# dfm/george

Hardware: NVIDIA H100
Metric: gp.compute+log_likelihood N-points/sec (higher is better)
Workload: dtype f64

## Files before the change

george_b200/csrc/hodlr.cu:

```cuda
#include <algorithm>
#include <cmath>
#include <cstdlib>
#include <cstring>
#include <vector>

#include "common.cuh"
#include "hodlr_kernels.cuh"
#include "hodlr_lu.cuh"
#include "hodlr_aca2.cuh"
#include "hodlr_leaf.cuh"
#include "linalg.cuh"
#include "kernel_eval.cuh"

namespace bgp {
int upload_program(const DevProgram& P, DevBuf<DevProgram>& buf, cudaStream_t s);
int kmat_grad_contract_launch(const DevProgram* dprog, int nd, int np, const unsigned* which_dev, const double* x,
                              int64_t n, const double* M, int64_t ldm, const double* alpha, double ca, double cm,
                              double* g_dev, double* diag_dev, DevBuf<double>& scratch, cudaStream_t s);
int fill_identity_launch(double* A, int64_t n, cudaStream_t s);
int64_t grad_slab_partial_size(int64_t n, int64_t c, int np);
int64_t grad_slab_tile_size(int64_t n, int np);
int kmat_grad_slab_launch(const DevProgram* dprog, int nd, int np, const unsigned* which_dev, const double* x, int64_t n,
                          const double* W, int64_t j0, int64_t nc, int64_t jlo, int64_t jhi, const double* alpha,
                          double* partial, double* tile_part, double* diag_dev, cudaStream_t s);
int kmat_grad_slab_finish(int np, int64_t jlo, int64_t jhi, const double* tile_part, double* g_dev, cudaStream_t s);
int kmat_symmetric_launch_auto(const DevProgram& P, const DevProgram* dprog, const double* x, int64_t n,
                               const double* diag_add, double* out, int64_t ld, cudaStream_t s);
int kmat_general_launch_auto(const DevProgram& P, const DevProgram* dprog, const double* x1, int64_t n1, const double* x2,
                             int64_t n2, double* out, int64_t ld, cudaStream_t s);
int kmat_diagonal_launch(const DevProgram* dprog, const double* x1, const double* x2, int64_t n, double* out,
                         cudaStream_t s, int members = 1, int64_t ostride = 0);
int64_t predict_chunk_cols(int64_t n, int64_t multiple);
int64_t predict_var_partial_size(int64_t n, int64_t c);
int predict_var_launch(const double* B, int64_t ldb, const double* W, int64_t ldw, int64_t n, int64_t c,
                       const double* kdiag, double* var, DevBuf<double>& scratch, cudaStream_t s);
int kmat_x1_grad_matvec_launch(const DevProgram& P, const DevProgram* dprog, const double* x1, int64_t n1,
                               const double* x2, int64_t n2, const double* V, int64_t ldv, double scale, int add_prior,
                               double* out, DevBuf<double>& scratch, cudaStream_t s);
int64_t x1_grad_partial_size(int64_t n1, int64_t n2, int nd);
void predict_gemm_plan(int64_t m, int64_t nn, int64_t K, int64_t* nsplit_out, int64_t* klen_out);
int predict_gemm_sub(const double* A, int64_t lda, const double* B, int64_t ldb, int64_t m, int64_t nn, int64_t K,
                     bool lower, double* C, int64_t ldc, DevBuf<double>& slices, DevBuf<GemmDesc>& descs, cudaStream_t s);
bool comm_ready();
int comm_rank();
int comm_world();
int comm_allreduce_sum_f64(double* buf, size_t count, cudaStream_t s);
int comm_allgather_f64(const double* send, double* recv, size_t count, cudaStream_t s);
}
using namespace bgp;

struct HNode {
  int start, size, half, is_leaf, parent, dir, depth;
  int slot;
  int rank = 0, draws = 0, fallback = 0;
  int owned = 1;
  int top = 0;
};

struct PanelSet {
  DevBuf<double> V, U;
  int64_t ld = 0, row_off = 0;
  int vcols = 0, ucols = 0;
  double* vbase() const { return V.p - row_off; }
  double* ubase() const { return U.p - row_off; }
};

struct LevelInfo {
  std::vector<int> nodes;
  int set = 1;
  int cap = 0, max_cap = 0, vcol = 0, r = 0, ucol = 0;
  int max_half = 0, grow = 0;
  int desc_off = 0;
};

struct AcaGraphKey {
  A2Args a;
  int nn, ncc, nrc, shape, grid;
};

struct bgp_hodlr {
  cudaStream_t sA = nullptr, sB = nullptr;
  cudaEvent_t ev[8] = {nullptr};
  int64_t n = 0;
  int ndim = 0;
  bgp_hodlr_opts_t opts;
  bool computed = false;
  double log_det = 0.0;
  DevProgram prog;

  std::vector<HNode> nodes;
  std::vector<int> leaves;
  std::vector<LevelInfo> levels;
  std::vector<int> piv_off;
  std::vector<int> h_piv_rows, h_piv_cols;
  int max_leaf = 0, rtot = 0, vcols = 0, cut_depth = 0;
  int64_t row0 = 0, nloc = 0;
  std::vector<int64_t> shard_row0, shard_rows;
  bool top_pending = false;

  DevBuf<DevProgram> d_prog;
  DevBuf<double> d_x, d_yerr, d_diag, d_L, d_leaf_logdet, d_node_logdet, d_S, d_W, d_scalar, d_rhs;
  PanelSet top, loc;
  const PanelSet& pset(const LevelInfo& L) const { return L.set == 0 ? top : loc; }
  DevBuf<double> d_inv, d_gscratch;
  DevBuf<double> d_xsend, d_xrecv;
  DevBuf<unsigned> d_which;
  LuWorkspace lu_ws;
  DevBuf<GemmDesc> d_gram_desc, d_upd_desc;
  std::vector<NodeDesc> h_nodes;
  std::vector<int> cap_hint;
  int64_t cap_hint_n = -1;
  int cap_hint_min_size = -1;
  DevBuf<LeafDesc> d_leaves;
  DevBuf<AcaDesc> d_aca;
  DevBuf<AcaOut> d_aca_out;
  DevBuf<NodeDesc> d_nodes;
  DevBuf<PanelTile> d_ptiles;
  int small_limit = SS_MAX_N;
  bool leaf_cols_wide = false;
  DevBuf<int> d_idx, d_piv_rows, d_piv_cols, d_ticket, d_chain_done, d_ncols_by_depth;
  DevBuf<uint32_t> d_chain_state;
  DevBuf<A2Node> d_a2nodes;
  DevBuf<A2State> d_a2states;
  DevBuf<MT19937> d_a2rngs;
  DevBuf<A2EPart> d_epart;
  DevBuf<int> d_cand, d_cand_k, d_cand_words, d_cand_L, d_cand_next, d_cand_live, d_cchunk_node, d_rchunk_node, d_nactive;
  DevBuf<double> d_node_box;
  DevBuf<double2> d_cand_xu, d_gbox, d_cbox;
  DevBuf<unsigned long long> d_cmax, d_stats;
  DevBuf<int4> d_work;
  DevBuf<int> d_work_count, d_iter;
  AcaGraphKey aca_key;
  cudaGraph_t aca_graph = nullptr;
  cudaGraphExec_t aca_exec = nullptr;
  cudaStream_t sC = nullptr;
  bool profile = false;
  std::vector<cudaEvent_t> prof_events;
  double prof[12] = {0, 0, 0, 0, 0, 0, 0, 0, 0, 0, 0, 0};
  uint64_t draw_paths[4] = {0, 0, 0, 0};
  uint64_t eval_units[2] = {0, 0};
  DevBuf<double> d_vpart, d_upart, d_vmax;
  int aca_iters = 0;
  size_t w_cap = 0;

  double t_ms[5] = {0, 0, 0, 0, 0};
  double grad_t[4] = {0, 0, 0, 0};
  double work[6] = {0, 0, 0, 0, 0, 0};
};

static int ensure_streams(bgp_hodlr* h) {
  if (!h->sA) {
    BGP_CUDA(cudaStreamCreateWithFlags(&h->sA, cudaStreamNonBlocking));
    BGP_CUDA(cudaStreamCreateWithFlags(&h->sB, cudaStreamNonBlocking));
    for (int i = 0; i < 8; ++i) BGP_CUDA(cudaEventCreate(&h->ev[i]));
  }
  return BGP_OK;
}

static void build_tree(bgp_hodlr* h, int start, int size, int dir, int parent, int depth) {
  HNode nd;
  nd.start = start; nd.size = size; nd.half = size / 2; nd.dir = dir; nd.parent = parent; nd.depth = depth;
  nd.is_leaf = !(nd.half >= h->opts.min_size);
  nd.slot = 0;
  const int id = (int)h->nodes.size();
  h->nodes.push_back(nd);
  if (!nd.is_leaf) {
    build_tree(h, start, nd.half, 0, id, depth + 1);
    build_tree(h, start + nd.half, size - nd.half, 1, id, depth + 1);
  }
}

static int hodlr_solve_dev(bgp_hodlr* h, double* b, int64_t nrhs, int64_t ldb, cudaStream_t s, int part,
                           int64_t eye_row0 = -1);
static int hodlr_exchange_finish(bgp_hodlr* h);

static bool host_exchange(const bgp_hodlr* h) {
  return h->opts.shard_count > 1 &&
         !(comm_ready() && comm_world() == h->opts.shard_count && comm_rank() == h->opts.shard_rank);
}

static int reject_host_exchange(const bgp_hodlr* h, const char* what) {
  if (!host_exchange(h)) return BGP_OK;
  set_error("%s is not available on a host-exchange shard (shard %d of %d without a matching communicator): use "
            "bgp_hodlr_solve_local_dev / bgp_hodlr_solve_top_dev", what, h->opts.shard_rank, h->opts.shard_count);
  return BGP_ERR_INVALID;
}
static int hodlr_finish_top_impl(bgp_hodlr* h, bool allreduce);

constexpr size_t LS_SMEM_MAX = 200 * 1024;
constexpr int LS_MAX_LEAF = (int)(LS_SMEM_MAX / sizeof(double));

static bool leaf_solve_fits(int max_leaf, int cols) { return sizeof(double) * (size_t)max_leaf * cols <= LS_SMEM_MAX; }

static void set_sweep_func_attrs() {
  static std::atomic<uint64_t> done{0};
  int dev = 0;
  cudaGetDevice(&dev);
  const uint64_t bit = dev < 64 ? (1ull << dev) : 0;
  if (bit && (done.load(std::memory_order_relaxed) & bit)) return;
  cudaFuncSetAttribute(leaf_solve_kernel<1>, cudaFuncAttributeMaxDynamicSharedMemorySize, (int)LS_SMEM_MAX);
  cudaFuncSetAttribute(leaf_solve_kernel<2>, cudaFuncAttributeMaxDynamicSharedMemorySize, (int)LS_SMEM_MAX);
  cudaFuncSetAttribute(leaf_solve_kernel<4>, cudaFuncAttributeMaxDynamicSharedMemorySize, (int)LS_SMEM_MAX);
  cudaFuncSetAttribute(leaf_solve_kernel<LS_COLS>, cudaFuncAttributeMaxDynamicSharedMemorySize, (int)LS_SMEM_MAX);
  cudaFuncSetAttribute(leaf_solve_kernel<LS_COLS_WIDE>, cudaFuncAttributeMaxDynamicSharedMemorySize, (int)LS_SMEM_MAX);
  cudaFuncSetAttribute(small_solve_kernel, cudaFuncAttributeMaxDynamicSharedMemorySize, 160 * 1024);
  done.fetch_or(bit, std::memory_order_relaxed);
}

template <int COLS>
static int leaf_solve_launch(bgp_hodlr* h, double* X, int64_t ldx, const int* ncols_by_depth, int ncols_fixed,
                             int max_cols, cudaStream_t s, int l0, int l1) {
  const int ngroups = (max_cols + COLS - 1) / COLS;
  const dim3 grid((unsigned)((size_t)(l1 - l0) * (size_t)ngroups));
  const size_t smem = sizeof(double) * (size_t)h->max_leaf * COLS;
  leaf_solve_kernel<COLS><<<grid, LS_THREADS, smem, s>>>(h->d_leaves.p + l0, h->d_L.p, X, ldx, ncols_by_depth,
                                                         ncols_fixed, h->max_leaf, ngroups);
  BGP_LAUNCH_CHECK();
  return BGP_OK;
}

static int launch_leaf_solve(bgp_hodlr* h, double* X, int64_t ldx, const int* ncols_by_depth, int ncols_fixed,
                             int max_cols, cudaStream_t s, int l0 = 0, int l1 = -1) {
  if (l1 < 0) l1 = (int)h->leaves.size();
  const int nl = l1 - l0;
  if (nl <= 0 || max_cols == 0) return BGP_OK;
  const int m = h->max_leaf;
  if (h->leaf_cols_wide && max_cols > LS_COLS && leaf_solve_fits(m, LS_COLS_WIDE))
    return leaf_solve_launch<LS_COLS_WIDE>(h, X, ldx, ncols_by_depth, ncols_fixed, max_cols, s, l0, l1);
  int cols = max_cols <= 1 ? 1 : max_cols <= 2 ? 2 : max_cols <= 4 ? 4 : LS_COLS;
  while (cols > 1 && !leaf_solve_fits(m, cols)) cols /= 2;
  if (!leaf_solve_fits(m, cols)) {
    set_error("leaf size %d too large for the leaf solve kernel (at most %d rows)", m, LS_MAX_LEAF);
    return BGP_ERR_INVALID;
  }
  switch (cols) {
    case LS_COLS: return leaf_solve_launch<LS_COLS>(h, X, ldx, ncols_by_depth, ncols_fixed, max_cols, s, l0, l1);
    case 4: return leaf_solve_launch<4>(h, X, ldx, ncols_by_depth, ncols_fixed, max_cols, s, l0, l1);
    case 2: return leaf_solve_launch<2>(h, X, ldx, ncols_by_depth, ncols_fixed, max_cols, s, l0, l1);
    default: return leaf_solve_launch<1>(h, X, ldx, ncols_by_depth, ncols_fixed, max_cols, s, l0, l1);
  }
}

static int launch_level_big(bgp_hodlr* h, const LevelInfo& L, double* X, int64_t ldx, int ncolsW, int own_off, int factor,
                            int col_lo, int col_hi, cudaStream_t s, int b0, int b1);

static int launch_level(bgp_hodlr* h, const LevelInfo& L, double* X, int64_t ldx, int ncolsW, int own_off, int factor,
                        int col_lo, int col_hi, cudaStream_t s, int b0 = 0, int b1 = -1) {
  if (b1 < 0) b1 = (int)L.nodes.size();
  const int nn = b1 - b0;
  if (nn <= 0 || L.r == 0) {
    return BGP_OK;
  }
  const int r = L.r;
  const int64_t stride = (int64_t)2 * r * ncolsW;
  const size_t need = (size_t)nn * stride;
  if (need > h->w_cap) { set_error("internal: W workspace too small (%zu > %zu)", need, h->w_cap); return BGP_ERR_CUDA; }
  BGP_CUDA(cudaMemsetAsync(h->d_W.p, 0, sizeof(double) * need, s));
  if (2 * r > h->small_limit) return launch_level_big(h, L, X, ldx, ncolsW, own_off, factor, col_lo, col_hi, s, b0, b1);
  const NodeDesc* nd = h->d_nodes.p + L.desc_off + b0;
  const int max_nh = L.max_half + 1;
  if (r <= GTS_MAX_R) {
    dim3 grid((max_nh + GTS_ROWS - 1) / GTS_ROWS, nn * 2, (ncolsW + GTS_TC - 1) / GTS_TC);
    const double* vb = h->pset(L).vbase();
    const int64_t ldv = h->pset(L).ld;
    if (r <= 2) gram_tn_small_kernel<2><<<grid, GTS_THREADS, 0, s>>>(nd, vb, ldv, X, ldx, ncolsW, h->d_W.p, stride);
    else if (r <= 4) gram_tn_small_kernel<4><<<grid, GTS_THREADS, 0, s>>>(nd, vb, ldv, X, ldx, ncolsW, h->d_W.p, stride);
    else gram_tn_small_kernel<GTS_MAX_R><<<grid, GTS_THREADS, 0, s>>>(nd, vb, ldv, X, ldx, ncolsW, h->d_W.p, stride);
    BGP_LAUNCH_CHECK();
  } else {
    dim3 grid((max_nh + GT_CHUNK - 1) / GT_CHUNK, nn * 2, (ncolsW + GT_TC - 1) / GT_TC);
    gram_tn_kernel<<<grid, GT_THREADS, 0, s>>>(nd, h->pset(L).vbase(), h->pset(L).ld, X, ldx, ncolsW, h->d_W.p, stride);
    BGP_LAUNCH_CHECK();
  }
  {
    const size_t sbytes = sizeof(double) * (size_t)(2 * r) * (2 * r);
    small_solve_kernel<<<nn, SS_THREADS, sbytes, s>>>(nd, h->d_W.p, stride, ncolsW, own_off, factor, h->d_S.p,
                                                      h->d_node_logdet.p, L.desc_off + b0);
    BGP_LAUNCH_CHECK();
  }
  if (col_hi > col_lo) {
    dim3 grid((max_nh + UP_ROWS - 1) / UP_ROWS, nn * 2, (col_hi - col_lo + UP_TC - 1) / UP_TC);
    update_nn_kernel<<<grid, UP_THREADS, 0, s>>>(nd, h->pset(L).ubase(), h->pset(L).ld, X, ldx, col_lo, col_hi, h->d_W.p, stride, 0);
    BGP_LAUNCH_CHECK();
  }
  return BGP_OK;
}

static int launch_level_big(bgp_hodlr* h, const LevelInfo& L, double* X, int64_t ldx, int ncolsW, int own_off, int factor,
                            int col_lo, int col_hi, cudaStream_t s, int b0, int b1) {
  const int nn = b1 - b0;
  const int r = L.r, n2 = 2 * r;
  const int64_t stride = (int64_t)n2 * ncolsW;
  const int64_t ldv = h->pset(L).ld, ldu = h->pset(L).ld;
  double* W = h->d_W.p;
  constexpr int KCHUNK = 4096;
  std::vector<LuNode> lun(nn);
  std::vector<GemmDesc> gram, upd;
  int max_nh = 0;
  for (int k = 0; k < nn; ++k) {
    const int b = b0 + k;
    const HNode& nd = h->nodes[L.nodes[b]];
    const int64_t s_off = h->h_nodes[L.desc_off + b].s_off;
    lun[k].S = h->d_S.p + s_off;
    lun[k].piv = reinterpret_cast<int*>(lun[k].S + (int64_t)n2 * n2);
    lun[k].logdet = h->d_node_logdet.p + L.desc_off + b;
    double* Wn = W + (int64_t)k * stride;
    for (int hh = 0; hh < 2; ++hh) {
      const int rs = nd.start + (hh ? nd.half : 0), nh = hh ? (nd.size - nd.half) : nd.half;
      max_nh = std::max(max_nh, nh);
      for (int k0 = 0; k0 < nh; k0 += KCHUNK) {
        GemmDesc g;
        g.A = h->pset(L).vbase() + (int64_t)L.vcol * ldv + rs + k0; g.lda = ldv;
        g.B = X + rs + k0; g.ldb = ldx;
        g.C = Wn + (hh ? 0 : r); g.ldc = n2;
        g.M = r; g.N = ncolsW; g.K = std::min(KCHUNK, nh - k0); g.mode = GD_ATOMIC_ADD;
        gram.push_back(g);
      }
      if (col_hi > col_lo) {
        GemmDesc g;
        g.A = h->pset(L).ubase() + (int64_t)L.ucol * ldu + rs; g.lda = ldu;
        g.B = Wn + (hh ? r : 0) + (int64_t)col_lo * n2; g.ldb = n2;
        g.C = X + rs + (int64_t)col_lo * ldx; g.ldc = ldx;
        g.M = nh; g.N = col_hi - col_lo; g.K = r; g.mode = GD_SUB;
        upd.push_back(g);
      }
    }
  }
  BGP_TRY(lu_upload(h->d_gram_desc, gram, s));
  BGP_TRY((gemm_dmma_launch<true, true>(h->d_gram_desc.p, (int)gram.size(), r, ncolsW, nullptr, s)));
  if (factor) {
    BGP_TRY(lu_upload(h->lu_ws.d_nodes, lun, s));
    dim3 grid((unsigned)std::min<int64_t>(((int64_t)n2 * n2 + 255) / 256, 4096), nn);
    lu_assemble_kernel<<<grid, 256, 0, s>>>(h->lu_ws.d_nodes.p, W, stride, r, own_off);
    BGP_LAUNCH_CHECK();
    BGP_TRY(lu_factor_batch(h->lu_ws, lun, n2, s));
    if (col_hi > col_lo)
      BGP_TRY(lu_solve_batch(h->lu_ws, lun, n2, W + (int64_t)col_lo * n2, stride, n2, col_hi - col_lo, false, s));
  } else {
    BGP_TRY(lu_solve_batch(h->lu_ws, lun, n2, W, stride, n2, ncolsW, true, s));
  }
  if (!upd.empty()) {
    BGP_TRY(lu_upload(h->d_upd_desc, upd, s));
    BGP_TRY((gemm_dmma_launch<false, true>(h->d_upd_desc.p, (int)upd.size(), max_nh, col_hi - col_lo, nullptr, s)));
  }
  return BGP_OK;
}

static int run_aca2(bgp_hodlr* h, const std::vector<AcaDesc>& descs, std::vector<AcaOut>& houts, cudaStream_t s) {
  const int nn = (int)descs.size();
  if (nn == 0) return BGP_OK;
  std::vector<A2Node> hn(nn);
  std::vector<int> cchunk_node, rchunk_node;
  int64_t cand_total = 0, top_cand_total = 0;
  (void)top_cand_total;
  const bool dist_top = false;
  int capmax = 1;
  for (int i = 0; i < nn; ++i) {
    const AcaDesc& d = descs[i];
    A2Node& a = hn[i];
    a.row0 = d.row0; a.n_rows = d.n_rows; a.col0 = d.col0; a.n_cols = d.n_cols;
    a.vcol = d.vcol; a.cap = d.cap; a.pre_id = d.pre_id; a.node = d.node;
    {
      const PanelSet& ps = h->pset(h->levels[h->nodes[d.pre_id].depth]);
      a.ld = ps.ld;
      a.vbase = ps.vbase() + (int64_t)d.vcol * ps.ld;
    }
    a.idx_off = d.idx_off; a.piv_off = d.piv_off;
    a.cchunk0 = (int)cchunk_node.size(); a.n_cchunks = (d.n_cols + A2_CHUNK - 1) / A2_CHUNK;
    a.rchunk0 = (int)rchunk_node.size(); a.n_rchunks = (d.n_rows + A2_CHUNK - 1) / A2_CHUNK;
    for (int c = 0; c < a.n_cchunks; ++c) cchunk_node.push_back(i);
    for (int c = 0; c < a.n_rchunks; ++c) rchunk_node.push_back(i);
    a.bmax = std::min(A2_BMAX, d.n_rows);
    a.cand_off = cand_total; cand_total += a.bmax;
    a.is_top = (dist_top && h->nodes[d.pre_id].top) ? 1 : 0;
    if (a.is_top) top_cand_total = cand_total;
    capmax = std::max(capmax, d.cap);
  }
  const int ncc = (int)cchunk_node.size(), nrc = (int)rchunk_node.size();
  BGP_TRY(h->d_a2nodes.reserve(nn, s));
  BGP_TRY(h->d_a2states.reserve(nn, s));
  BGP_TRY(h->d_a2rngs.reserve((size_t)2 * nn, s));
  BGP_TRY(h->d_cand.reserve((size_t)cand_total, s));
  BGP_TRY(h->d_cand_k.reserve((size_t)cand_total, s));
  BGP_TRY(h->d_cand_words.reserve((size_t)cand_total, s));
  BGP_TRY(h->d_cand_L.reserve((size_t)cand_total, s));
  BGP_TRY(h->d_cand_next.reserve((size_t)cand_total, s));
  BGP_TRY(h->d_cand_live.reserve((size_t)cand_total, s));
  BGP_TRY(h->d_node_box.reserve((size_t)2 * nn, s));
  BGP_TRY(h->d_cmax.reserve((size_t)cand_total, s));
  BGP_TRY(h->d_epart.reserve((size_t)std::max(ncc, 1) * A2_NSUB, s));
  BGP_TRY(h->d_cchunk_node.reserve(ncc, s));
  BGP_TRY(h->d_rchunk_node.reserve(nrc, s));
  BGP_TRY(h->d_vpart.reserve((size_t)ncc * A2_NSUB * (capmax + 1), s));
  BGP_TRY(h->d_upart.reserve((size_t)nrc * A2_NSUB * (capmax + 1), s));
  const bool cull = shape_has_bound(h->prog.shape) && !getenv("BGP_NO_CULL");
  if (cull) {
    BGP_TRY(h->d_vmax.reserve((size_t)ncc * A2_NGROUP, s));
    BGP_CUDA(cudaMemsetAsync(h->d_vmax.p, 0, sizeof(double) * ncc * A2_NGROUP, s));
    BGP_TRY(h->d_cand_xu.reserve((size_t)cand_total, s));
    BGP_TRY(h->d_gbox.reserve((size_t)ncc * A2_NGROUP, s));
    BGP_TRY(h->d_cbox.reserve((size_t)ncc, s));
  }
  BGP_TRY(h->d_nactive.reserve(2, s));
  int n_top = 0;
  for (int i = 0; i < nn; ++i) n_top += hn[i].is_top;
  BGP_TRY(h->d_stats.reserve(A2_NSTATS, s));
  int64_t work_cap = 0;
  for (int i = 0; i < nn; ++i) {
    const int big = (hn[i].bmax + A2_CG * A2_ITEM_CB - 1) / (A2_CG * A2_ITEM_CB);
    const int small = (std::min(hn[i].bmax, 256) + A2_CG - 1) / A2_CG;
    work_cap += (int64_t)hn[i].n_cchunks * std::max(big, small);
  }
  BGP_TRY(h->d_work.reserve((size_t)(2 * work_cap), s));
  BGP_TRY(h->d_work_count.reserve(4, s));
  BGP_TRY(h->d_iter.reserve(1, s));
  BGP_CUDA(cudaMemsetAsync(h->d_iter.p, 0, sizeof(int), s));
  BGP_CUDA(cudaMemsetAsync(h->d_work_count.p, 0, sizeof(int) * 4, s));
  BGP_CUDA(cudaMemsetAsync(h->d_stats.p, 0, sizeof(unsigned long long) * A2_NSTATS, s));
  BGP_CUDA(cudaMemcpyAsync(h->d_a2nodes.p, hn.data(), sizeof(A2Node) * nn, cudaMemcpyHostToDevice, s));
  BGP_CUDA(cudaMemcpyAsync(h->d_cchunk_node.p, cchunk_node.data(), sizeof(int) * ncc, cudaMemcpyHostToDevice, s));
  BGP_CUDA(cudaMemcpyAsync(h->d_rchunk_node.p, rchunk_node.data(), sizeof(int) * nrc, cudaMemcpyHostToDevice, s));
  BGP_CUDA(cudaMemcpyAsync(h->d_nactive.p, &nn, sizeof(int), cudaMemcpyHostToDevice, s));
  A2Args a;
  memset(&a, 0, sizeof(a));
  a.prog = h->d_prog.p; a.x = h->d_x.p; a.nodes = h->d_a2nodes.p; a.states = h->d_a2states.p; a.rngs = h->d_a2rngs.p; a.n_nodes = nn;
  a.tol = h->opts.tol; a.seed = (uint32_t)h->opts.seed; a.exhaust_mode = h->opts.exhaust_mode;
  a.idx_ws = h->d_idx.p; a.piv_rows = h->d_piv_rows.p; a.piv_cols = h->d_piv_cols.p;
  a.cand = h->d_cand.p; a.cand_k = h->d_cand_k.p; a.cand_words = h->d_cand_words.p; a.cmax = h->d_cmax.p; a.epart = h->d_epart.p;
  a.cchunk_node = h->d_cchunk_node.p; a.rchunk_node = h->d_rchunk_node.p; a.vpart = h->d_vpart.p; a.upart = h->d_upart.p;
  a.vmax = cull ? h->d_vmax.p : nullptr;
  a.cand_xu = cull ? h->d_cand_xu.p : nullptr;
  a.gbox = cull ? h->d_gbox.p : nullptr;
  a.cbox = cull ? h->d_cbox.p : nullptr;
  a.cand_L = h->d_cand_L.p; a.cand_next = h->d_cand_next.p; a.cand_live = h->d_cand_live.p; a.node_box = h->d_node_box.p;
  a.capmax = capmax; a.n_active = h->d_nactive.p; a.stats = h->d_stats.p;
  a.work = h->d_work.p; a.work_count = h->d_work_count.p; a.work_cursor = h->d_work_count.p + 2; a.work_cap = (int)work_cap; a.iter_ptr = h->d_iter.p;
  a.shard_rank = dist_top ? h->opts.shard_rank : 0; a.shard_count = dist_top ? h->opts.shard_count : 1;
  if (dist_top) BGP_CUDA(cudaMemcpyAsync(h->d_nactive.p + 1, &n_top, sizeof(int), cudaMemcpyHostToDevice, s));
  cudaFuncSetAttribute(a2_init_kernel, cudaFuncAttributeMaxDynamicSharedMemorySize, (int)sizeof(A2NodeSmem));
    cudaFuncSetAttribute(a2_decide_kernel, cudaFuncAttributeMaxDynamicSharedMemorySize, (int)sizeof(A2NodeSmem));
    cudaFuncSetAttribute(a2_finish_kernel, cudaFuncAttributeMaxDynamicSharedMemorySize, (int)sizeof(A2NodeSmem));
  a2_init_kernel<<<nn, A2_NODE_THREADS, sizeof(A2NodeSmem), s>>>(a);
  BGP_LAUNCH_CHECK();
  int active = nn, iters = 0;
  int eval_minb = A2_EVAL_MINB_DEFAULT;
  if (const char* e = getenv("BGP_EVAL_MINB")) eval_minb = atoi(e) == 3 ? 3 : 2;
  const int eval_grid = num_sms() * 6;
  auto launch_iteration = [&](cudaStream_t st, cudaGraphConditionalHandle hnd, int use_hnd, int it_prof) -> int {
    auto mark = [&](int slot) -> int {
      if (it_prof < 0) return BGP_OK;
      const size_t need = (size_t)7 * (it_prof + 1);
      while (h->prof_events.size() < need) {
        cudaEvent_t e;
        BGP_CUDA(cudaEventCreate(&e));
        h->prof_events.push_back(e);
      }
      BGP_CUDA(cudaEventRecord(h->prof_events[(size_t)7 * it_prof + slot], st));
      return BGP_OK;
    };
    BGP_TRY(mark(0));
    a2_eval_launch(h->prog.shape, dim3(eval_grid), st, a, eval_minb);
    BGP_LAUNCH_CHECK();
    BGP_TRY(mark(1));
    a2_decide_kernel<<<nn, A2_NODE_THREADS, sizeof(A2NodeSmem), st>>>(a);
    BGP_LAUNCH_CHECK();
    BGP_TRY(mark(2));
    a2_vrow_launch(h->prog.shape, dim3(ncc, A2_NSUB), st, a);
    BGP_LAUNCH_CHECK();
    BGP_TRY(mark(3));
    a2_pivot_kernel<<<nn, 32, 0, st>>>(a);
    BGP_LAUNCH_CHECK();
    BGP_TRY(mark(4));
    a2_vnorm_ucol_launch(h->prog.shape, dim3(ncc + nrc, A2_NSUB), st, a, ncc);
    BGP_LAUNCH_CHECK();
    BGP_TRY(mark(5));
    a2_finish_kernel<<<nn, A2_NODE_THREADS, sizeof(A2NodeSmem), st>>>(a);
    BGP_LAUNCH_CHECK();
    BGP_TRY(mark(6));
    a2_tick_kernel<<<1, 1, 0, st>>>(a.iter_ptr, a.n_active, hnd, use_hnd);
    BGP_LAUNCH_CHECK();
    return BGP_OK;
  };
  const bool use_graph = !h->profile && !getenv("BGP_NO_GRAPH");
  if (use_graph) {
    AcaGraphKey key;
    memset(&key, 0, sizeof(key));
    key.a = a; key.nn = nn; key.ncc = ncc; key.nrc = nrc; key.shape = h->prog.shape; key.grid = eval_grid * 4 + eval_minb;
    if (!h->aca_exec || memcmp(&key, &h->aca_key, sizeof(key)) != 0) {
      if (h->aca_exec) { cudaGraphExecDestroy(h->aca_exec); h->aca_exec = nullptr; }
      if (h->aca_graph) { cudaGraphDestroy(h->aca_graph); h->aca_graph = nullptr; }
      BGP_CUDA(cudaGraphCreate(&h->aca_graph, 0));
      cudaGraphConditionalHandle hnd;
      BGP_CUDA(cudaGraphConditionalHandleCreate(&hnd, h->aca_graph, 1, cudaGraphCondAssignDefault));
      cudaGraphNodeParams cp = {};
      cp.type = cudaGraphNodeTypeConditional;
      cp.conditional.handle = hnd;
      cp.conditional.type = cudaGraphCondTypeWhile;
      cp.conditional.size = 1;
      cudaGraphNode_t wnode;
      BGP_CUDA(cudaGraphAddNode(&wnode, h->aca_graph, nullptr, 0, &cp));
      cudaGraph_t body = cp.conditional.phGraph_out[0];
      if (!h->sC) BGP_CUDA(cudaStreamCreateWithFlags(&h->sC, cudaStreamNonBlocking));
      BGP_CUDA(cudaStreamBeginCaptureToGraph(h->sC, body, nullptr, nullptr, 0, cudaStreamCaptureModeRelaxed));
      const int rc = launch_iteration(h->sC, hnd, 1, -1);
      cudaGraph_t captured = nullptr;
      const cudaError_t ce = cudaStreamEndCapture(h->sC, &captured);
      if (rc != BGP_OK) return rc;
      if (ce != cudaSuccess) { set_error("ACA graph capture failed: %s", cudaGetErrorString(ce)); return BGP_ERR_CUDA; }
      BGP_CUDA(cudaGraphInstantiate(&h->aca_exec, h->aca_graph, 0));
      h->aca_key = key;
    }
    BGP_CUDA(cudaGraphLaunch(h->aca_exec, s));
    int it_host = 0, act2[2] = {0, 0};
    BGP_CUDA(cudaMemcpyAsync(&it_host, h->d_iter.p, sizeof(int), cudaMemcpyDeviceToHost, s));
    BGP_CUDA(cudaMemcpyAsync(act2, h->d_nactive.p, sizeof(int) * 2, cudaMemcpyDeviceToHost, s));
    BGP_CUDA(cudaStreamSynchronize(s));
    iters = it_host;
// ... 1329 lines not shown
```

george_b200/csrc/hodlr_kernels.cuh:

```cuda
#pragma once

#include <cooperative_groups.h>

#include "common.cuh"
#include "kernel_eval.cuh"

namespace bgp {

namespace cg = cooperative_groups;

struct MT19937 {
  uint32_t mt[624];
  int idx;
};
__device__ inline void mt_seed(MT19937& g, uint32_t s) {
  g.mt[0] = s;
  for (int i = 1; i < 624; ++i) g.mt[i] = 1812433253u * (g.mt[i - 1] ^ (g.mt[i - 1] >> 30)) + (uint32_t)i;
  g.idx = 624;
}
__device__ inline uint32_t mt_next(MT19937& g) {
  if (g.idx >= 624) {
    for (int i = 0; i < 624; ++i) {
      const uint32_t y = (g.mt[i] & 0x80000000u) | (g.mt[(i + 1) % 624] & 0x7fffffffu);
      g.mt[i] = g.mt[(i + 397) % 624] ^ (y >> 1) ^ ((y & 1u) ? 0x9908b0dfu : 0u);
    }
    g.idx = 0;
  }
  uint32_t y = g.mt[g.idx++];
  y ^= (y >> 11);
  y ^= (y << 7) & 0x9d2c5680u;
  y ^= (y << 15) & 0xefc60000u;
  y ^= (y >> 18);
  return y;
}
__device__ inline int mt_uniform(MT19937& g, uint32_t s, int* words) {
  uint64_t prod = (uint64_t)mt_next(g) * (uint64_t)s;
  uint32_t low = (uint32_t)prod;
  int w = 1;
  if (low < s) {
    const uint32_t thr = (0u - s) % s;
    while (low < thr) {
      prod = (uint64_t)mt_next(g) * (uint64_t)s;
      low = (uint32_t)prod;
      ++w;
    }
  }
  *words += w;
  return (int)(prod >> 32);
}
__host__ __device__ inline uint32_t node_seed(uint32_t seed, int pre_id) { return seed + 0x9E3779B9u * (uint32_t)pre_id; }

struct LeafDesc {
  int start, size, depth, _pad;
  int64_t off;
};

constexpr int LEAF_THREADS = 256;
constexpr int LEAF_NB = 32;

__global__ void __launch_bounds__(LEAF_THREADS) leaf_build_factor_kernel(const DevProgram* __restrict__ gprog,
                                                                         const double* __restrict__ x,
                                                                         const double* __restrict__ diag,
                                                                         const LeafDesc* __restrict__ leaves,
                                                                         double* __restrict__ Lbuf,
                                                                         double* __restrict__ leaf_logdet) {
  __shared__ DevProgram P;
  __shared__ double red[32];
  __shared__ double panel[LEAF_NB][LEAF_NB + 1];
  __shared__ double dinv[LEAF_NB];
  stage_program(&P, gprog);
  __syncthreads();
  const LeafDesc lf = leaves[blockIdx.x];
  const int m = lf.size, nd = P.ndim;
  double* A = Lbuf + lf.off;
  const double* xs = x + (int64_t)lf.start * nd;

  for (int j = 0; j < m; ++j) {
    for (int i = j + threadIdx.x; i < m; i += LEAF_THREADS) {
      double v = kernel_value(P, xs + (int64_t)i * nd, xs + (int64_t)j * nd);
      if (i == j) v += diag[lf.start + i];
      A[(int64_t)j * m + i] = v;
    }
  }
  __syncthreads();

  double logdet = 0.0;
  for (int k0 = 0; k0 < m; k0 += LEAF_NB) {
    const int nb = min(LEAF_NB, m - k0);
    for (int t = threadIdx.x; t < nb * nb; t += LEAF_THREADS) {
      const int i = t % nb, j = t / nb;
      panel[i][j] = (i >= j) ? A[(int64_t)(k0 + j) * m + k0 + i] : 0.0;
    }
    __syncthreads();
    for (int k = 0; k < nb; ++k) {
      const double d = panel[k][k];
      const double inv = 1.0 / d;
      __syncthreads();
      for (int i = k + 1 + threadIdx.x; i < nb; i += LEAF_THREADS) panel[i][k] *= inv;
      __syncthreads();
      for (int t = threadIdx.x; t < (nb - k - 1) * (nb - k - 1); t += LEAF_THREADS) {
        const int i = k + 1 + t % (nb - k - 1), j = k + 1 + t / (nb - k - 1);
        if (i >= j) panel[i][j] -= panel[i][k] * d * panel[j][k];
      }
      __syncthreads();
    }
    if (threadIdx.x < nb) {
      const double d = panel[threadIdx.x][threadIdx.x];
      dinv[threadIdx.x] = 1.0 / d;
      logdet += log(fabs(d));
    }
    for (int t = threadIdx.x; t < nb * nb; t += LEAF_THREADS) {
      const int i = t % nb, j = t / nb;
      if (i >= j) A[(int64_t)(k0 + j) * m + k0 + i] = panel[i][j];
    }
    __syncthreads();
    const int rem = m - k0 - nb;
    if (rem <= 0) break;
    for (int i = threadIdx.x; i < rem; i += LEAF_THREADS) {
      double* row = A + k0 + nb + i;
      double w[LEAF_NB];
#pragma unroll
      for (int j = 0; j < LEAF_NB; ++j) w[j] = (j < nb) ? row[(int64_t)(k0 + j) * m] : 0.0;
#pragma unroll
      for (int j = 0; j < LEAF_NB; ++j) {
        if (j < nb) {
          double s = w[j];
#pragma unroll
          for (int q = 0; q < j; ++q) s -= w[q] * panel[j][q];
          w[j] = s;
        }
      }
#pragma unroll
      for (int j = 0; j < LEAF_NB; ++j)
        if (j < nb) row[(int64_t)(k0 + j) * m] = w[j] * dinv[j];
    }
    __syncthreads();
    {
      const int tiles = (rem + 3) / 4;
      const double* Lp = A + (int64_t)k0 * m + k0 + nb;
      for (int t = threadIdx.x; t < tiles * tiles; t += LEAF_THREADS) {
        const int ti = t % tiles, tj = t / tiles;
        if (ti < tj) continue;
        double acc[4][4];
#pragma unroll
        for (int a = 0; a < 4; ++a)
#pragma unroll
          for (int b = 0; b < 4; ++b) acc[a][b] = 0.0;
        for (int q = 0; q < nb; ++q) {
          const double dq = panel[q][q];
          double li[4], lj[4];
#pragma unroll
          for (int a = 0; a < 4; ++a) {
            const int i = ti * 4 + a, j = tj * 4 + a;
            li[a] = (i < rem) ? Lp[(int64_t)q * m + i] : 0.0;
            lj[a] = (j < rem) ? Lp[(int64_t)q * m + j] * dq : 0.0;
          }
#pragma unroll
          for (int a = 0; a < 4; ++a)
#pragma unroll
            for (int b = 0; b < 4; ++b) acc[a][b] += li[a] * lj[b];
        }
#pragma unroll
        for (int b = 0; b < 4; ++b)
#pragma unroll
          for (int a = 0; a < 4; ++a) {
            const int i = ti * 4 + a, j = tj * 4 + b;
            if (i < rem && j < rem && i >= j) A[(int64_t)(k0 + nb + j) * m + k0 + nb + i] -= acc[a][b];
          }
      }
    }
    __syncthreads();
  }
  logdet = block_sum(logdet, red);
  if (threadIdx.x == 0) leaf_logdet[blockIdx.x] = logdet;
}

constexpr int LS_THREADS = 256;
constexpr int LS_COLS = 8;
constexpr int LS_COLS_WIDE = 32;
constexpr int LS_NB = 32;
constexpr int LS_BATCH = 4;

template <int COLS>
__global__ void __launch_bounds__(LS_THREADS, COLS <= LS_COLS ? 3 : 1) leaf_solve_kernel(const LeafDesc* __restrict__ leaves,
                                                                const double* __restrict__ Lbuf,
                                                                double* __restrict__ X, int64_t ldx,
                                                                const int* __restrict__ ncols_by_depth, int ncols_fixed,
                                                                int max_m, int ngroups) {
  extern __shared__ double xs[];
  __shared__ double sL[LS_NB][LS_NB + 1];
  const LeafDesc lf = leaves[blockIdx.x / ngroups];
  const int ncols = ncols_by_depth ? ncols_by_depth[lf.depth] : ncols_fixed;
  const int c0 = (blockIdx.x % ngroups) * COLS;
  if (c0 >= ncols) return;
  const int nc = min(COLS, ncols - c0);
  const int m = lf.size;
  const double* A = Lbuf + lf.off;
  const int lane = threadIdx.x & 31, warp = threadIdx.x >> 5;
  constexpr int NW = LS_THREADS / 32;
  for (int t = threadIdx.x; t < m * COLS; t += LS_THREADS) {
    const int i = t % m, c = t / m;
    xs[c * max_m + i] = (c < nc) ? X[(int64_t)(c0 + c) * ldx + lf.start + i] : 0.0;
  }
  for (int kb = 0; kb < m; kb += LS_NB) {
    const int nb = min(LS_NB, m - kb);
    __syncthreads();
    for (int t = threadIdx.x; t < LS_NB * LS_NB; t += LS_THREADS) {
      const int i = t % LS_NB, k = t / LS_NB;
      sL[i][k] = (i < nb && k < nb && i > k) ? A[(int64_t)(kb + k) * m + kb + i] : 0.0;
    }
    __syncthreads();
    for (int c = warp; c < nc; c += NW) {
      double y = (lane < nb) ? xs[c * max_m + kb + lane] : 0.0;
      for (int k = 0; k < nb; ++k) {
        const double yk = __shfl_sync(0xffffffffu, y, k);
        if (lane > k) y -= sL[lane][k] * yk;
      }
      if (lane < nb) xs[c * max_m + kb + lane] = y;
    }
    __syncthreads();
    const int r0 = kb + nb;
    for (int i = r0 + threadIdx.x; i < m; i += LS_THREADS) {
      double acc[COLS];
#pragma unroll
      for (int c = 0; c < COLS; ++c) acc[c] = 0.0;
      const double* Li = A + (int64_t)kb * m + i;
#pragma unroll 8
      for (int k = 0; k < nb; ++k) {
        const double l = Li[(int64_t)k * m];
#pragma unroll
        for (int c = 0; c < COLS; ++c) acc[c] += l * xs[c * max_m + kb + k];
      }
#pragma unroll
      for (int c = 0; c < COLS; ++c) if (c < nc) xs[c * max_m + i] -= acc[c];
    }
  }
  __syncthreads();
  for (int t = threadIdx.x; t < m * nc; t += LS_THREADS) {
    const int i = t % m, c = t / m;
    xs[c * max_m + i] /= A[(int64_t)i * m + i];
  }
  const int nblk = (m + LS_NB - 1) / LS_NB;
  for (int b = nblk - 1; b >= 0; --b) {
    const int kb = b * LS_NB;
    const int nb = min(LS_NB, m - kb);
    const int r0 = kb + nb;
    __syncthreads();
    for (int t = threadIdx.x; t < LS_NB * LS_NB; t += LS_THREADS) {
      const int i = t % LS_NB, k = t / LS_NB;
      sL[i][k] = (i < nb && k < nb && i > k) ? A[(int64_t)(kb + k) * m + kb + i] : 0.0;
    }
    for (int k = warp; k < nb; k += NW) {
      double acc[COLS];
#pragma unroll
      for (int c = 0; c < COLS; ++c) acc[c] = 0.0;
      const double* Lk = A + (int64_t)(kb + k) * m;
      for (int i0 = r0 + lane; i0 < m; i0 += 32 * LS_BATCH) {
        double l[LS_BATCH];
#pragma unroll
        for (int j = 0; j < LS_BATCH; ++j) l[j] = (i0 + 32 * j < m) ? Lk[i0 + 32 * j] : 0.0;
#pragma unroll
        for (int j = 0; j < LS_BATCH; ++j) {
          const int i = i0 + 32 * j;
          if (i < m) {
#pragma unroll
            for (int c = 0; c < COLS; ++c) acc[c] += l[j] * xs[c * max_m + i];
          }
        }
      }
#pragma unroll
      for (int c = 0; c < COLS; ++c) {
        const double sres = warp_sum(acc[c]);
        if (lane == 0 && c < nc) xs[c * max_m + kb + k] -= sres;
      }
    }
    __syncthreads();
    for (int c = warp; c < nc; c += NW) {
      double y = (lane < nb) ? xs[c * max_m + kb + lane] : 0.0;
      for (int k = nb - 1; k >= 0; --k) {
        const double zk = __shfl_sync(0xffffffffu, y, k);
        if (lane < k) y -= sL[k][lane] * zk;
      }
      if (lane < nb) xs[c * max_m + kb + lane] = y;
    }
  }
  __syncthreads();
  for (int t = threadIdx.x; t < m * nc; t += LS_THREADS) {
    const int i = t % m, c = t / m;
    X[(int64_t)(c0 + c) * ldx + lf.start + i] = xs[c * max_m + i];
  }
}

struct AcaDesc {
  int row0, n_rows, col0, n_cols;
  int vcol, cap, pre_id, node;
  int64_t idx_off;
  int64_t piv_off;
};
struct AcaOut {
  int rank, draws, fallback, status;
};

constexpr int ACA_THREADS = 512;
constexpr int ACA_MAX_NDIM = 32;

struct AcaShared {
  DevProgram P;
  MT19937 rng;
  double red[32];
  int redi[32];
  double xpiv[ACA_MAX_NDIM];
  double bc[4];
  int ibc[4];
};

__device__ __forceinline__ void block_argmax(double& v, int& i, double* red, int* redi) {
  const int lane = threadIdx.x & 31, w = threadIdx.x >> 5, nw = (blockDim.x + 31) >> 5;
  warp_argmax(v, i);
  __syncthreads();
  if (lane == 0) { red[w] = v; redi[w] = i; }
  __syncthreads();
  double tv = (lane < nw) ? red[lane] : -1.0;
  int ti = (lane < nw) ? redi[lane] : 0x7fffffff;
  warp_argmax(tv, ti);
  v = tv; i = ti;
}
__device__ __forceinline__ double block_max(double v, double* red) {
  const int lane = threadIdx.x & 31, w = threadIdx.x >> 5, nw = (blockDim.x + 31) >> 5;
  v = warp_max(v);
  __syncthreads();
  if (lane == 0) red[w] = v;
  __syncthreads();
  double t = (lane < nw) ? red[lane] : 0.0;
  return warp_max(t);
}

__device__ __forceinline__ double block_max_signed(double v, double* red) {
  const int lane = threadIdx.x & 31, w = threadIdx.x >> 5, nw = (blockDim.x + 31) >> 5;
  v = warp_max(v);
  __syncthreads();
  if (lane == 0) red[w] = v;
  __syncthreads();
  double t = (lane < nw) ? red[lane] : -__longlong_as_double(0x7ff0000000000000ll);
  return warp_max(t);
}

__global__ void __launch_bounds__(ACA_THREADS) aca_kernel(const DevProgram* __restrict__ gprog,
                                                          const double* __restrict__ x,
                                                          const AcaDesc* __restrict__ descs, int n_desc,
                                                          double* __restrict__ Vp, int64_t ld, double tol,
                                                          uint32_t seed, int rng_mode, int* __restrict__ idx_ws,
                                                          int* __restrict__ piv_rows, int* __restrict__ piv_cols,
                                                          AcaOut* __restrict__ outs, int* __restrict__ ticket,
                                                          uint32_t* chain_state, volatile int* chain_done,
                                                          int exhaust_mode) {
  extern __shared__ __align__(16) unsigned char aca_smem_raw[];
  AcaShared* S = reinterpret_cast<AcaShared*>(aca_smem_raw);
  double* rowbuf = reinterpret_cast<double*>(aca_smem_raw + ((sizeof(AcaShared) + 15) & ~size_t(15)));
  __shared__ int s_ticket;

  stage_program(&S->P, gprog);
  if (threadIdx.x == 0) s_ticket = atomicAdd(ticket, 1);
  __syncthreads();
  const int tk = s_ticket;
  if (tk >= n_desc) return;
  const AcaDesc d = descs[tk];
  const int nd = S->P.ndim;
  const int n_rows = d.n_rows, n_cols = d.n_cols;
  const int max_rank = min(n_rows, n_cols);
  int* index = idx_ws + d.idx_off;
  double* Vcols = Vp + (int64_t)d.vcol * ld;
  const double* xr = x + (int64_t)d.row0 * nd;
  const double* xc = x + (int64_t)d.col0 * nd;

  for (int n = threadIdx.x; n < n_rows; n += blockDim.x) index[n] = n;
  if (threadIdx.x == 0) {
    if (rng_mode == BGP_RNG_REFERENCE) {
      if (tk > 0) {
        while (chain_done[tk - 1] == 0) __nanosleep(200);
        __threadfence();
        for (int i = 0; i < 624; ++i) S->rng.mt[i] = chain_state[i];
        S->rng.idx = (int)chain_state[624];
      } else {
        mt_seed(S->rng, seed);
      }
    } else {
      mt_seed(S->rng, node_seed(seed, d.pre_id));
    }
  }
  __syncthreads();

  int rank = 0, draws = 0, n_index = n_rows, fallback = 0, status = 0;
  double norm = 0.0;
  const double tol2 = tol * tol;

  while (true) {
    int i = 0, j = 0;
    double pivot = 0.0;
    bool exhausted = false;
    if (rank >= d.cap) { status = 1; break; }
    while (true) {
      if (n_index == 0) { exhausted = true; break; }
      if (threadIdx.x == 0) {
        int w = 0;
        const int k = mt_uniform(S->rng, (uint32_t)n_index, &w);
        const int ii = index[k];
        index[k] = index[n_index - 1];
        S->ibc[0] = ii;
        S->ibc[1] = w;
      }
      __syncthreads();
      i = S->ibc[0];
      draws += S->ibc[1];
      n_index--;
      for (int k = threadIdx.x; k < rank; k += blockDim.x) rowbuf[k] = __ldcg(Vcols + (int64_t)k * ld + d.row0 + i);
      for (int q = threadIdx.x; q < nd; q += blockDim.x) S->xpiv[q] = xr[(int64_t)i * nd + q];
      __syncthreads();
      double best = -1.0;
      int bidx = 0x7fffffff;
      double* vnew = Vcols + (int64_t)rank * ld + d.col0;
      for (int n = threadIdx.x; n < n_cols; n += blockDim.x) {
        double val = kernel_value(S->P, S->xpiv, xc + (int64_t)n * nd);
        const double* vk = Vcols + d.col0 + n;
        int k = 0;
        for (; k + 4 <= rank; k += 4) {
          const double a0 = vk[(int64_t)(k + 0) * ld], a1 = vk[(int64_t)(k + 1) * ld];
          const double a2 = vk[(int64_t)(k + 2) * ld], a3 = vk[(int64_t)(k + 3) * ld];
          val -= rowbuf[k] * a0;
          val -= rowbuf[k + 1] * a1;
          val -= rowbuf[k + 2] * a2;
          val -= rowbuf[k + 3] * a3;
        }
        for (; k < rank; ++k) val -= rowbuf[k] * vk[(int64_t)k * ld];
        vnew[n] = val;
        const double a = aca_pivot_key(val);
        if (a > best) { best = a; bidx = n; }
      }
      block_argmax(best, bidx, S->red, S->redi);
      j = bidx;
      __syncthreads();
      pivot = vnew[j];
      if (!(fabs(pivot) < 1e-14)) break;
    }
    if (exhausted) {
      fallback = 1;
      if (exhaust_mode == BGP_EXHAUST_LOWRANK) break;
      if (max_rank > d.cap) { status = 1; rank = 0; break; }
      for (int mcol = 0; mcol < n_cols; ++mcol) {
        double* vc = Vcols + (int64_t)mcol * ld;
        for (int n = threadIdx.x; n < n_cols; n += blockDim.x) vc[d.col0 + n] = (n == mcol) ? 1.0 : 0.0;
        for (int n = threadIdx.x; n < n_rows; n += blockDim.x)
          vc[d.row0 + n] = kernel_value(S->P, xr + (int64_t)n * nd, xc + (int64_t)mcol * nd);
      }
      rank = max_rank;
      break;
    }
    double* vnew = Vcols + (int64_t)rank * ld + d.col0;
    double vn2 = 0.0;
    for (int n = threadIdx.x; n < n_cols; n += blockDim.x) {
      const double v = vnew[n] / pivot;
      vnew[n] = v;
      vn2 += v * v;
    }
    vn2 = block_sum(vn2, S->red);
    double vdot = 0.0;
    {
      const int warp = threadIdx.x >> 5, lane = threadIdx.x & 31, nw = blockDim.x >> 5;
      for (int k = warp; k < rank; k += nw) {
        const double* vk = Vcols + (int64_t)k * ld + d.col0;
        double s = 0.0;
        for (int n = lane; n < n_cols; n += 32) s += vk[n] * vnew[n];
        s = warp_sum(s);
        vdot = fmax(vdot, fabs(s));
      }
      vdot = block_max(vdot, S->red);
    }
    for (int k = threadIdx.x; k < rank; k += blockDim.x) rowbuf[k] = __ldcg(Vcols + (int64_t)k * ld + d.col0 + j);
    for (int q = threadIdx.x; q < nd; q += blockDim.x) S->xpiv[q] = xc[(int64_t)j * nd + q];
    __syncthreads();
    double* unew = Vcols + (int64_t)rank * ld + d.row0;
    double un2 = 0.0;
    for (int n = threadIdx.x; n < n_rows; n += blockDim.x) {
      double val = kernel_value(S->P, xr + (int64_t)n * nd, S->xpiv);
      const double* uk = Vcols + d.row0 + n;
      int k = 0;
      for (; k + 4 <= rank; k += 4) {
        const double a0 = uk[(int64_t)(k + 0) * ld], a1 = uk[(int64_t)(k + 1) * ld];
        const double a2 = uk[(int64_t)(k + 2) * ld], a3 = uk[(int64_t)(k + 3) * ld];
        val -= rowbuf[k] * a0;
        val -= rowbuf[k + 1] * a1;
        val -= rowbuf[k + 2] * a2;
        val -= rowbuf[k + 3] * a3;
      }
      for (; k < rank; ++k) val -= rowbuf[k] * uk[(int64_t)k * ld];
      unew[n] = val;
      un2 += val * val;
    }
    un2 = block_sum(un2, S->red);
    double udot = 0.0;
    {
      const int warp = threadIdx.x >> 5, lane = threadIdx.x & 31, nw = blockDim.x >> 5;
      for (int k = warp; k < rank; k += nw) {
        const double* uk = Vcols + (int64_t)k * ld + d.row0;
        double s = 0.0;
        for (int n = lane; n < n_rows; n += 32) s += uk[n] * unew[n];
        s = warp_sum(s);
        udot = fmax(udot, fabs(s));
      }
      udot = block_max(udot, S->red);
    }
    if (threadIdx.x == 0) { piv_rows[d.piv_off + rank] = i; piv_cols[d.piv_off + rank] = j; }
    rank++;
    if (rank >= max_rank) break;
    const double rowcol = un2 * vn2;
    if (rowcol < tol2 * norm) break;
    norm += rowcol;
    if (rank > 1) norm += 2.0 * udot + 2.0 * vdot;
  }

  __syncthreads();
  if (threadIdx.x == 0) {
    AcaOut o;
    o.rank = rank; o.draws = draws; o.fallback = fallback; o.status = status;
    outs[d.node] = o;
    if (rng_mode == BGP_RNG_REFERENCE) {
      for (int q = 0; q < 624; ++q) chain_state[q] = S->rng.mt[q];
      chain_state[624] = (uint32_t)S->rng.idx;
      __threadfence();
      chain_done[tk] = 1;
    }
  }
}

struct NodeDesc {
  int start, size, half, depth;
  int vcol;
  int ucol;
  int r;
  int rank;
  int64_t s_off;
};

struct PanelTile {
  int node;
  int row0;
};

constexpr int FP_THREADS = 256;
constexpr int FP_ROWS = 1024;

__global__ void __launch_bounds__(FP_THREADS) finalize_panels_kernel(const NodeDesc* __restrict__ nodes,
                                                                     const PanelTile* __restrict__ tiles,
                                                                     double* __restrict__ Vp, int64_t ldv,
                                                                     double* __restrict__ Up, int64_t ldu) {
  const PanelTile t = tiles[blockIdx.x];
  const NodeDesc nd = nodes[t.node];
  const int row_hi = min(nd.size, t.row0 + FP_ROWS);
  for (int k = 0; k < nd.r; ++k) {
    double* v = Vp + (int64_t)(nd.vcol + k) * ldv + nd.start;
    double* u = Up + (int64_t)(nd.ucol + k) * ldu + nd.start;
    const bool used = k < nd.rank;
#pragma unroll
    for (int e = 0; e < FP_ROWS / FP_THREADS; ++e) {
      const int i = t.row0 + e * FP_THREADS + threadIdx.x;
      if (i < row_hi) {
        double val = 0.0;
        if (used) val = v[i]; else v[i] = 0.0;
        u[i] = val;
      }
    }
  }
}

constexpr int GT_THREADS = 256;
constexpr int GT_ROWS = 64;
constexpr int GT_TQ = 32;
constexpr int GT_TC = 32;
constexpr int GT_CHUNK = 512;

__global__ void __launch_bounds__(GT_THREADS) gram_tn_kernel(const NodeDesc* __restrict__ nodes,
                                                             const double* __restrict__ Vp, int64_t ldv,
                                                             const double* __restrict__ X, int64_t ldx, int ncols,
                                                             double* __restrict__ W, int64_t w_stride_node) {
  __shared__ double sv[GT_ROWS][GT_TQ + 1];
  __shared__ double sx[GT_ROWS][GT_TC + 1];
  const NodeDesc nd = nodes[blockIdx.y >> 1];
// ... 327 lines not shown
```

Baseline: 23.56 million.

## Double-buffer leaf-solve triangle tiles with cp.async and register-prefetch panel loads

Restructures the leaf triangular solve kernel so the diagonal 32x32 tile is copied into a double-buffered shared-memory area with cp.async while the current block is processed. The off-diagonal panel update now prefetches 16 L entries per thread into registers, with two half-warps splitting the k range and combining via shuffle, instead of streaming column loads. The backward sweep gets the same register-tiled update with shuffle reductions, in place of per-warp row dot products. Dynamic shared memory grows to hold the two tiles and a staging vector, which may reduce occupancy, and the code adds register pressure.

```diff
diff --git a/george_b200/csrc/hodlr.cu b/george_b200/csrc/hodlr.cu
--- a/george_b200/csrc/hodlr.cu
+++ b/george_b200/csrc/hodlr.cu
@@ -191,6 +191,7 @@
 constexpr int LS_MAX_LEAF = (int)(LS_SMEM_MAX / sizeof(double));
 
 static bool leaf_solve_fits(int max_leaf, int cols) { return sizeof(double) * (size_t)max_leaf * cols <= LS_SMEM_MAX; }
+static int ls_smem_limit(int cols) { return (int)(LS_SMEM_MAX + ls_smem_bytes(0, cols)); }
 
 static void set_sweep_func_attrs() {
   static std::atomic<uint64_t> done{0};
@@ -198,11 +199,12 @@
   cudaGetDevice(&dev);
   const uint64_t bit = dev < 64 ? (1ull << dev) : 0;
   if (bit && (done.load(std::memory_order_relaxed) & bit)) return;
-  cudaFuncSetAttribute(leaf_solve_kernel<1>, cudaFuncAttributeMaxDynamicSharedMemorySize, (int)LS_SMEM_MAX);
-  cudaFuncSetAttribute(leaf_solve_kernel<2>, cudaFuncAttributeMaxDynamicSharedMemorySize, (int)LS_SMEM_MAX);
-  cudaFuncSetAttribute(leaf_solve_kernel<4>, cudaFuncAttributeMaxDynamicSharedMemorySize, (int)LS_SMEM_MAX);
-  cudaFuncSetAttribute(leaf_solve_kernel<LS_COLS>, cudaFuncAttributeMaxDynamicSharedMemorySize, (int)LS_SMEM_MAX);
-  cudaFuncSetAttribute(leaf_solve_kernel<LS_COLS_WIDE>, cudaFuncAttributeMaxDynamicSharedMemorySize, (int)LS_SMEM_MAX);
+  cudaFuncSetAttribute(leaf_solve_kernel<1>, cudaFuncAttributeMaxDynamicSharedMemorySize, ls_smem_limit(1));
+  cudaFuncSetAttribute(leaf_solve_kernel<2>, cudaFuncAttributeMaxDynamicSharedMemorySize, ls_smem_limit(2));
+  cudaFuncSetAttribute(leaf_solve_kernel<4>, cudaFuncAttributeMaxDynamicSharedMemorySize, ls_smem_limit(4));
+  cudaFuncSetAttribute(leaf_solve_kernel<LS_COLS>, cudaFuncAttributeMaxDynamicSharedMemorySize, ls_smem_limit(LS_COLS));
+  cudaFuncSetAttribute(leaf_solve_kernel<LS_COLS_WIDE>, cudaFuncAttributeMaxDynamicSharedMemorySize,
+                       ls_smem_limit(LS_COLS_WIDE));
   cudaFuncSetAttribute(small_solve_kernel, cudaFuncAttributeMaxDynamicSharedMemorySize, 160 * 1024);
   done.fetch_or(bit, std::memory_order_relaxed);
 }
@@ -212,7 +214,7 @@
                              int max_cols, cudaStream_t s, int l0, int l1) {
   const int ngroups = (max_cols + COLS - 1) / COLS;
   const dim3 grid((unsigned)((size_t)(l1 - l0) * (size_t)ngroups));
-  const size_t smem = sizeof(double) * (size_t)h->max_leaf * COLS;
+  const size_t smem = ls_smem_bytes(h->max_leaf, COLS);
   leaf_solve_kernel<COLS><<<grid, LS_THREADS, smem, s>>>(h->d_leaves.p + l0, h->d_L.p, X, ldx, ncols_by_depth,
                                                          ncols_fixed, h->max_leaf, ngroups);
   BGP_LAUNCH_CHECK();
diff --git a/george_b200/csrc/hodlr_kernels.cuh b/george_b200/csrc/hodlr_kernels.cuh
--- a/george_b200/csrc/hodlr_kernels.cuh
+++ b/george_b200/csrc/hodlr_kernels.cuh
@@ -3,6 +3,7 @@
 #include <cooperative_groups.h>
 
 #include "common.cuh"
+#include "gemm_dmma.cuh"
 #include "kernel_eval.cuh"
 
 namespace bgp {
@@ -179,7 +180,12 @@
 constexpr int LS_COLS = 8;
 constexpr int LS_COLS_WIDE = 32;
 constexpr int LS_NB = 32;
-constexpr int LS_BATCH = 4;
+constexpr int LS_LDT = LS_NB + 1;
+constexpr int LS_KB = 16;
+
+__host__ __device__ inline size_t ls_smem_bytes(int max_m, int cols) {
+  return sizeof(double) * ((size_t)max_m * cols + 2 * LS_NB * LS_LDT + (size_t)LS_NB * cols);
+}
 
 template <int COLS>
 __global__ void __launch_bounds__(LS_THREADS, COLS <= LS_COLS ? 3 : 1) leaf_solve_kernel(const LeafDesc* __restrict__ leaves,
@@ -188,7 +194,8 @@
                                                                 const int* __restrict__ ncols_by_depth, int ncols_fixed,
                                                                 int max_m, int ngroups) {
   extern __shared__ double xs[];
-  __shared__ double sL[LS_NB][LS_NB + 1];
+  double* const sT = xs + (size_t)max_m * COLS;
+  double* const sy = sT + 2 * LS_NB * LS_LDT;
   const LeafDesc lf = leaves[blockIdx.x / ngroups];
   const int ncols = ncols_by_depth ? ncols_by_depth[lf.depth] : ncols_fixed;
   const int c0 = (blockIdx.x % ngroups) * COLS;
@@ -197,42 +204,63 @@
   const int m = lf.size;
   const double* A = Lbuf + lf.off;
   const int lane = threadIdx.x & 31, warp = threadIdx.x >> 5;
-  constexpr int NW = LS_THREADS / 32;
+  const int nblk = (m + LS_NB - 1) / LS_NB;
   for (int t = threadIdx.x; t < m * COLS; t += LS_THREADS) {
     const int i = t % m, c = t / m;
     xs[c * max_m + i] = (c < nc) ? X[(int64_t)(c0 + c) * ldx + lf.start + i] : 0.0;
   }
-  for (int kb = 0; kb < m; kb += LS_NB) {
-    const int nb = min(LS_NB, m - kb);
-    __syncthreads();
-    for (int t = threadIdx.x; t < LS_NB * LS_NB; t += LS_THREADS) {
-      const int i = t % LS_NB, k = t / LS_NB;
-      sL[i][k] = (i < nb && k < nb && i > k) ? A[(int64_t)(kb + k) * m + kb + i] : 0.0;
-    }
-    __syncthreads();
-    for (int c = warp; c < nc; c += NW) {
+  auto copy_tile = [&](int b) {
+    const int kb = b * LS_NB, nb = min(LS_NB, m - kb);
+    double* T = sT + (b & 1) * LS_NB * LS_LDT;
+    for (int k = warp; k < LS_NB; k += LS_THREADS / 32) {
+      const bool valid = lane > k && lane < nb;
+      cp_async8(T + lane * LS_LDT + k, valid ? A + (int64_t)(kb + k) * m + kb + lane : A, valid);
+    }
+    cp_async_commit();
+  };
+  double l[LS_KB];
+
+  const int fh = lane >> 4, frow = warp * 16 + (lane & 15);
+  auto load_fwd = [&](int kb, int nb, int r) {
+#pragma unroll
+    for (int j = 0; j < LS_KB; ++j) {
+      const int k = fh * LS_KB + j;
+      l[j] = (r < m && k < nb) ? A[(int64_t)(kb + k) * m + r] : 0.0;
+    }
+  };
+  copy_tile(0);
+  for (int b = 0; b < nblk; ++b) {
+    const int kb = b * LS_NB, nb = min(LS_NB, m - kb), r0 = kb + nb;
+    const double* T = sT + (b & 1) * LS_NB * LS_LDT;
+    load_fwd(kb, nb, r0 + frow);
+    cp_async_wait<0>();
+    __syncthreads();
+    if (b + 1 < nblk) copy_tile(b + 1);
+    for (int c = warp; c < nc; c += LS_THREADS / 32) {
       double y = (lane < nb) ? xs[c * max_m + kb + lane] : 0.0;
       for (int k = 0; k < nb; ++k) {
         const double yk = __shfl_sync(0xffffffffu, y, k);
-        if (lane > k) y -= sL[lane][k] * yk;
-      }
-      if (lane < nb) xs[c * max_m + kb + lane] = y;
-    }
-    __syncthreads();
-    const int r0 = kb + nb;
-    for (int i = r0 + threadIdx.x; i < m; i += LS_THREADS) {
+        if (lane > k) y -= T[lane * LS_LDT + k] * yk;
+      }
+      if (lane < nb) { xs[c * max_m + kb + lane] = y; sy[c * LS_NB + lane] = y; }
+    }
+    __syncthreads();
+    for (int p = r0; p < m; p += LS_THREADS / 2) {
+      const int r = p + frow;
+      if (p > r0) load_fwd(kb, nb, r);
       double acc[COLS];
 #pragma unroll
       for (int c = 0; c < COLS; ++c) acc[c] = 0.0;
-      const double* Li = A + (int64_t)kb * m + i;
-#pragma unroll 8
-      for (int k = 0; k < nb; ++k) {
-        const double l = Li[(int64_t)k * m];
-#pragma unroll
-        for (int c = 0; c < COLS; ++c) acc[c] += l * xs[c * max_m + kb + k];
-      }
-#pragma unroll
-      for (int c = 0; c < COLS; ++c) if (c < nc) xs[c * max_m + i] -= acc[c];
+#pragma unroll
+      for (int j = 0; j < LS_KB; ++j)
+#pragma unroll
+        for (int c = 0; c < COLS; ++c) acc[c] += l[j] * sy[c * LS_NB + fh * LS_KB + j];
+#pragma unroll
+      for (int c = 0; c < COLS; ++c) acc[c] += __shfl_xor_sync(0xffffffffu, acc[c], 16);
+      if (fh == 0 && r < m) {
+#pragma unroll
+        for (int c = 0; c < COLS; ++c) if (c < nc) xs[c * max_m + r] -= acc[c];
+      }
     }
   }
   __syncthreads();
@@ -240,48 +268,52 @@
     const int i = t % m, c = t / m;
     xs[c * max_m + i] /= A[(int64_t)i * m + i];
   }
-  const int nblk = (m + LS_NB - 1) / LS_NB;
+  const int bk = warp * 4 + (lane & 3), brow = lane >> 2;
+  auto load_bwd = [&](int kb, int nb, int p) {
+#pragma unroll
+    for (int j = 0; j < LS_KB; ++j) {
+      const int r = p + brow + 8 * j;
+      l[j] = (r < m && bk < nb) ? A[(int64_t)(kb + bk) * m + r] : 0.0;
+    }
+  };
+  copy_tile(nblk - 1);
   for (int b = nblk - 1; b >= 0; --b) {
-    const int kb = b * LS_NB;
-    const int nb = min(LS_NB, m - kb);
-    const int r0 = kb + nb;
-    __syncthreads();
-    for (int t = threadIdx.x; t < LS_NB * LS_NB; t += LS_THREADS) {
-      const int i = t % LS_NB, k = t / LS_NB;
-      sL[i][k] = (i < nb && k < nb && i > k) ? A[(int64_t)(kb + k) * m + kb + i] : 0.0;
-    }
-    for (int k = warp; k < nb; k += NW) {
-      double acc[COLS];
-#pragma unroll
-      for (int c = 0; c < COLS; ++c) acc[c] = 0.0;
-      const double* Lk = A + (int64_t)(kb + k) * m;
-      for (int i0 = r0 + lane; i0 < m; i0 += 32 * LS_BATCH) {
-        double l[LS_BATCH];
-#pragma unroll
-        for (int j = 0; j < LS_BATCH; ++j) l[j] = (i0 + 32 * j < m) ? Lk[i0 + 32 * j] : 0.0;
-#pragma unroll
-        for (int j = 0; j < LS_BATCH; ++j) {
-          const int i = i0 + 32 * j;
-          if (i < m) {
-#pragma unroll
-            for (int c = 0; c < COLS; ++c) acc[c] += l[j] * xs[c * max_m + i];
-          }
+    const int kb = b * LS_NB, nb = min(LS_NB, m - kb), r0 = kb + nb;
+    const double* T = sT + (b & 1) * LS_NB * LS_LDT;
+    load_bwd(kb, nb, r0);
+    cp_async_wait<0>();
+    __syncthreads();
+    if (b > 0) copy_tile(b - 1);
+    double acc[COLS];
+#pragma unroll
+    for (int c = 0; c < COLS; ++c) acc[c] = 0.0;
+    for (int p = r0; p < m; p += 8 * LS_KB) {
+      if (p > r0) load_bwd(kb, nb, p);
+#pragma unroll
+      for (int j = 0; j < LS_KB; ++j) {
+        const int r = p + brow + 8 * j;
+        if (r < m) {
+#pragma unroll
+          for (int c = 0; c < COLS; ++c) acc[c] += l[j] * xs[c * max_m + r];
         }
       }
-#pragma unroll
-      for (int c = 0; c < COLS; ++c) {
-        const double sres = warp_sum(acc[c]);
-        if (lane == 0 && c < nc) xs[c * max_m + kb + k] -= sres;
-      }
-    }
-    __syncthreads();
-    for (int c = warp; c < nc; c += NW) {
-      double y = (lane < nb) ? xs[c * max_m + kb + lane] : 0.0;
+    }
+#pragma unroll
+    for (int off = 4; off < 32; off <<= 1)
+#pragma unroll
+      for (int c = 0; c < COLS; ++c) acc[c] += __shfl_xor_sync(0xffffffffu, acc[c], off);
+    if (brow == 0 && bk < nb) {
+#pragma unroll
+      for (int c = 0; c < COLS; ++c) sy[c * LS_NB + bk] = xs[c * max_m + kb + bk] - acc[c];
+    }
+    __syncthreads();
+    for (int c = warp; c < nc; c += LS_THREADS / 32) {
+      double z = (lane < nb) ? sy[c * LS_NB + lane] : 0.0;
       for (int k = nb - 1; k >= 0; --k) {
-        const double zk = __shfl_sync(0xffffffffu, y, k);
-        if (lane < k) y -= sL[k][lane] * zk;
-      }
-      if (lane < nb) xs[c * max_m + kb + lane] = y;
+        const double zk = __shfl_sync(0xffffffffu, z, k);
+        if (lane < k) z -= T[k * LS_LDT + lane] * zk;
+      }
+      if (lane < nb) xs[c * max_m + kb + lane] = z;
     }
   }
   __syncthreads();
```

Result: faster. 24.46 million, median of 6 (+3.8%).
